# viniciusvidal2/slam-sensor-fusion

Measured on AMD Instinct MI355X. Metric: scans_per_s_200k_scan_vs_10M_map, higher is better.
Workload: dtype f32 points / f64 accumulation

## Files before the change

### include/slamfusion.h

```cpp
#ifndef SLAMFUSION_H
#define SLAMFUSION_H
#include <stdint.h>

#ifdef __cplusplus
extern "C" {
#endif

#define SF_VERSION 210

typedef enum {
    SF_OK = 0,
    SF_ERR_INVALID = -1,
    SF_ERR_HIP = -2,
    SF_ERR_NOMEM = -3,
    SF_ERR_STATE = -4,
    SF_ERR_OVERFLOW = -5,
    SF_ERR_COMM = -6
} sf_status;

typedef struct sf_ctx sf_ctx;
typedef struct sf_cloud sf_cloud;
typedef struct sf_map sf_map;
typedef struct sf_icp sf_icp;

// ... 375 lines not shown
int sf_node_set_coarse_alignment_complete(sf_node *n, int complete);
int sf_node_coarse_alignment_complete(sf_node *n);
sf_icp *sf_node_icp(sf_node *n);
struct sf_bf;
struct sf_bf *sf_node_bf(sf_node *n);

typedef struct sf_ekf sf_ekf;
int sf_ekf_create(sf_ekf **out);
void sf_ekf_destroy(sf_ekf *e);
int sf_ekf_reset(sf_ekf *e, const double T[16], const double v[3] , const double P_diag[9] );
int sf_ekf_set_noise(sf_ekf *e, double gyro_sigma, double accel_sigma, const double gravity[3] );
int sf_ekf_set_bias(sf_ekf *e, const double gyro_bias[3], const double accel_bias[3], const double gyro_bias_var[3], const double accel_bias_var[3]);
int sf_ekf_set_bias_noise(sf_ekf *e, double gyro_bias_walk, double accel_bias_walk);
int sf_ekf_predict_imu(sf_ekf *e, const double *gyro, const double *accel, int64_t n, double dt);
int sf_ekf_predict_odometry(sf_ekf *e, const double odom_T_prev[16], const double odom_T_cur[16], const double cov_pos[3], const double cov_rot[3]);
int sf_ekf_update_position(sf_ekf *e, const double p_map[3], const double cov[9]);
int sf_ekf_update_yaw(sf_ekf *e, double yaw, double var);
int sf_ekf_update_pose(sf_ekf *e, const double T[16], const double cov_pos[3], const double cov_rot[3]);
int sf_ekf_update_pose_cov(sf_ekf *e, const double T[16], const double cov[36]);
int sf_ekf_get(const sf_ekf *e, double T[16], double v[3], double P[81]);
int sf_ekf_get_full(const sf_ekf *e, double gyro_bias[3], double accel_bias[3], double P[225]);

int sf_test_radix_sort(sf_ctx *ctx, int key_bytes , const void *keys, const uint32_t *vals , int64_t n, unsigned end_bit,
                       int lead , int lead_alt , void *keys_out, uint32_t *vals_out , int64_t *guard_damage);
int sf_test_scan_u32(sf_ctx *ctx, int op , const uint32_t *in, int64_t n, uint32_t carry0, int in_place, uint32_t *out,
                     int64_t *guard_damage);

#define SF_TEST_OP_RSQRT 0
#define SF_TEST_OP_SVD3 1
#define SF_TEST_OP_KABSCH 2
#define SF_TEST_OP_LDLT6 3
#define SF_TEST_OP_VEC6 4
#define SF_TEST_OP_JACOBI3 5
#define SF_TEST_OP_JACOBI6 6
#define SF_TEST_OP_ROBUST 7
#define SF_TEST_OP_EIGVEC 8
int sf_test_linalg(sf_ctx *ctx, int op, const double *in, int in_stride, int64_t cases, double *out, int out_stride);
int sf_test_wave_reduce(sf_ctx *ctx, int width , const double *in , double *out );
int sf_test_block_reduce(sf_ctx *ctx, int nrec , const double *in , double *out );
int sf_test_reduce_partials(sf_ctx *ctx, int nrec , int nt , const double *part , int nblocks, double *out );

int sf_test_plane_score(sf_cloud *c, const float *planes, int64_t n_planes, double t, int max_blocks, int64_t *counts);

int sf_test_label_boxes(sf_cloud *c, const int32_t *labels, int64_t n_labels, const sf_box_params *p, int max_blocks,
                        sf_label_box *boxes, sf_box_stats *stats);

#define SF_TEST_SCHEDULE_IN 15
#define SF_TEST_SCHEDULE_OUT 10
int sf_test_launch_schedule(const int32_t *in, int64_t rows, int k, int32_t *out);

int sf_test_compact(sf_cloud *c, const uint8_t *flags);
int sf_test_cloud_minmax(sf_cloud *c, int enqueue_form, float mn[3], float mx[3], int64_t *n_finite);

#ifdef __cplusplus
}
#endif
#endif
```

### slam_sensor_fusion_amd/api.py

```python
import atexit
import ctypes as C
import math
import os
import weakref

import numpy as np

_HERE = os.path.dirname(os.path.abspath(__file__))
LIB_PATH = os.path.join(_HERE, "lib", "libslamfusion.so")

SF_ICP_REF_CPP, SF_ICP_O3D_P2P, SF_ICP_P2PLANE = 0, 1, 2
SF_VOXEL_PCL, SF_VOXEL_O3D, SF_VOXEL_PCL64 = 0, 1, 2
SF_FLAG_VOXEL_OVERFLOW = 1
SF_ICP_FLAG_FEW_CORR, SF_ICP_FLAG_SINGULAR, SF_ICP_FLAG_SHARD_STALE, SF_ICP_FLAG_BARRIER_TIMEOUT = 1, 2, 4, 8
PROF_NN, PROF_REDUCE, PROF_COLLECTIVE, PROF_SOLVE, PROF_SHARD_BUILD = 0, 1, 2, 3, 4
SF_ERR_COMM = -6
MODES = {"ref_cpp": SF_ICP_REF_CPP, "o3d_p2p": SF_ICP_O3D_P2P, "p2plane": SF_ICP_P2PLANE}
ROBUST_KINDS = {"none": 0, "huber": 1, "cauchy": 2, "tukey": 3, "gm": 4}


class SlamFusionError(RuntimeError):
    pass


# ... 130 lines not shown


atexit.register(_close_all)


def load_library():
    global _lib
    if _lib is not None:
        return _lib
    if not os.path.exists(LIB_PATH):
        raise SlamFusionError(
            "libslamfusion.so not found at %s — build it with "
            "`python -c 'import __graft_entry__ as g; g.build()'` (hipcc, gfx950). "
            "There is no CPU fallback." % LIB_PATH)
    try:
        import torch
    except ImportError:
        pass
    lib = C.CDLL(LIB_PATH)
    lib.sf_last_error.restype = C.c_char_p
    lib.sf_ctx_stream.restype = C.c_void_p
    lib.sf_cloud_device_ptr.restype = C.c_void_p
    lib.sf_icp_exchange_ptr.restype = C.c_void_p
    lib.sf_sfilter_create.restype = C.c_void_p
    lib.sf_node_icp.restype = C.c_void_p
    lib.sf_node_bf.restype = C.c_void_p
    lib.sf_fusion_compass_to_yaw.restype = C.c_float
    lib.sf_fusion_closest_altitude.restype = C.c_float
    lib.sf_sfilter_pose_zscore.restype = C.c_float
    lib.sf_icp_set_robust_kernel.argtypes = [C.c_void_p, C.c_int, C.c_double]
    lib.sf_icp_set_covariance.argtypes = [C.c_void_p, C.c_int, C.c_double]
    lib.sf_icp_set_degeneracy_thresholds.argtypes = [C.c_void_p, C.c_double, C.c_double, C.c_double, C.c_double]
    lib.sf_icp_fetch_covariance.argtypes = [C.c_void_p, C.c_void_p]
    lib.sf_icp_fetch_covariance_previous.argtypes = [C.c_void_p, C.c_void_p]
    lib.sf_test_radix_sort.argtypes = [C.c_void_p, C.c_int, C.c_void_p, C.c_void_p, C.c_int64, C.c_uint, C.c_int, C.c_int, C.c_void_p, C.c_void_p, C.c_void_p]
    lib.sf_test_scan_u32.argtypes = [C.c_void_p, C.c_int, C.c_void_p, C.c_int64, C.c_uint32, C.c_int, C.c_void_p, C.c_void_p]
    lib.sf_test_linalg.argtypes = [C.c_void_p, C.c_int, C.c_void_p, C.c_int, C.c_int64, C.c_void_p, C.c_int]
    lib.sf_test_wave_reduce.argtypes = [C.c_void_p, C.c_int, C.c_void_p, C.c_void_p]
    lib.sf_test_block_reduce.argtypes = [C.c_void_p, C.c_int, C.c_void_p, C.c_void_p]
    lib.sf_test_reduce_partials.argtypes = [C.c_void_p, C.c_int, C.c_int, C.c_void_p, C.c_int, C.c_void_p]
    lib.sf_plane_default_params.restype = None
    lib.sf_cloud_plane_hypotheses.argtypes = [C.c_void_p, C.c_void_p, C.c_void_p, C.c_void_p, C.c_void_p]
    lib.sf_cloud_score_planes.argtypes = [C.c_void_p, C.c_void_p, C.c_int64, C.c_double, C.c_void_p]
    lib.sf_cloud_segment_plane.argtypes = [C.c_void_p, C.c_void_p, C.c_void_p, C.c_void_p, C.c_void_p]
    lib.sf_cloud_remove_plane.argtypes = [C.c_void_p, C.c_void_p, C.c_int, C.c_void_p, C.c_void_p]
    lib.sf_test_plane_score.argtypes = [C.c_void_p, C.c_void_p, C.c_int64, C.c_double, C.c_int, C.c_void_p]
    lib.sf_cloud_label_boxes.argtypes = [C.c_void_p, C.c_void_p, C.c_int64, C.c_void_p, C.c_void_p, C.c_void_p]
    lib.sf_test_label_boxes.argtypes = [C.c_void_p, C.c_void_p, C.c_int64, C.c_void_p, C.c_int, C.c_void_p, C.c_void_p]
    lib.sf_cloud_cluster_boxes.argtypes = [C.c_void_p, C.c_double, C.c_int64, C.c_int64, C.c_float, C.c_void_p, C.c_void_p, C.c_int64, C.c_void_p, C.c_void_p]
    lib.sf_cloud_remove_boxes.argtypes = [C.c_void_p, C.c_void_p, C.c_void_p, C.c_void_p, C.c_int64, C.c_double, C.c_int, C.c_void_p]
    lib.sf_test_launch_schedule.argtypes = [C.c_void_p, C.c_int64, C.c_int, C.c_void_p]
    lib.sf_test_compact.argtypes = [C.c_void_p, C.c_void_p]
    lib.sf_test_cloud_minmax.argtypes = [C.c_void_p, C.c_int, C.c_void_p, C.c_void_p, C.c_void_p]
    _lib = lib
    return lib


def voxel_merge_min_points(n=-1):
    return int(load_library().sf_cloud_voxel_merge_min_points(C.c_int64(n)))


def kernel_sources():
    import re
    csrc = os.path.join(_HERE, "csrc")
    found, todo = set(), ["sf_icp.hip"]
    while todo:
        name = todo.pop()
        if name in found or not os.path.isfile(os.path.join(csrc, name)):
            continue
        found.add(name)
        with open(os.path.join(csrc, name), "r", encoding="utf-8", errors="replace") as f:
            todo += re.findall(r'^[ \t]*#[ \t]*include[ \t]*"([^"]+)"', f.read(), re.M)
    return sorted(found)


def kernel_source_hash():
    import hashlib
    h = hashlib.sha256()
    for name in kernel_sources():
        with open(os.path.join(_HERE, "csrc", name), "rb") as f:
            h.update(f.read())
    return h.hexdigest()[:16]


def _check(rc):
    if rc != 0:
        raise SlamFusionError("libslamfusion error %d: %s" % (rc, load_library().sf_last_error().decode()))


def _f32(a):
    return np.ascontiguousarray(a, dtype=np.float32)


def _f64(a):
    return np.ascontiguousarray(a, dtype=np.float64)


def _p(a):
    return a.ctypes.data_as(C.c_void_p)


SCHEDULE_INPUTS = ("mode", "K", "qpl", "sharded", "whole", "reuse", "window", "robust", "wanted", "fz_from", "defer", "table", "nbr_from", "lk_min", "tile_on")
SCHEDULE_OUTPUTS = ("launches", "nn", "one_per_lane", "solve_takes_freeze_state", "ask_freeze", "deferred_rows", "attempt_from", "fz", "lookup_first", "defer_first")
NN_SEARCH, NN_TILE_SEARCH, NN_DEFERRING, NN_FREEZE, NN_FROZEN_FEW = range(5)


# ... 31 lines not shown
def hook_scan_u32(ctx, op, values, carry0=0, in_place=False):
    values = np.ascontiguousarray(values, dtype=np.uint32)
    out = np.empty_like(values)
    damage = C.c_int64(-1)
    _check(ctx.lib.sf_test_scan_u32(ctx.h, int(op), _p(values), len(values), int(carry0), int(bool(in_place)), _p(out), C.addressof(damage)))
    return out, damage.value


LINALG_OPS = {"rsqrt": (0, 1, 2), "svd3": (1, 9, 21), "kabsch": (2, 32, 16), "ldlt6": (3, 42, 7), "vec6": (4, 6, 16),
              "jacobi3": (5, 9, 13), "jacobi6": (6, 36, 43), "robust": (7, 3, 1), "eigvec": (8, 9, 3)}


def hook_linalg(ctx, op, cases):
    code, n_in, n_out = LINALG_OPS[op]
    cases = _f64(cases).reshape(-1, n_in)
    out = np.zeros((len(cases), n_out))
    _check(ctx.lib.sf_test_linalg(ctx.h, code, _p(cases), n_in, len(cases), _p(out), n_out))
    return out


def hook_wave_reduce(ctx, width, values):
    values = _f64(values).reshape(256, int(width))
    out = np.zeros(256)
    _check(ctx.lib.sf_test_wave_reduce(ctx.h, int(width), _p(values), _p(out)))
    return out


def hook_block_reduce(ctx, nrec, values, fill=0.0):
    values = _f64(values).reshape(256, int(nrec))
    out = np.full(32, fill, dtype=np.float64)
    _check(ctx.lib.sf_test_block_reduce(ctx.h, int(nrec), _p(values), _p(out)))
    return out


def hook_reduce_partials(ctx, nrec, nt, part):
    part = _f64(part).reshape(-1, 32)
    out = np.full(32, np.nan)
    _check(ctx.lib.sf_test_reduce_partials(ctx.h, int(nrec), int(nt), _p(part), len(part), _p(out)))
    return out


def hook_compact(cloud, flags):
    flags = np.ascontiguousarray(flags, dtype=np.uint8).reshape(-1)
    if len(flags) != len(cloud):
        raise SlamFusionError("hook_compact: %d flags for %d points" % (len(flags), len(cloud)))
    _check(cloud.lib.sf_test_compact(cloud.h, _p(flags) if len(flags) else None))
    return cloud.download(), cloud.last_indices()


def hook_cloud_minmax(cloud, enqueue=False):
    mn, mx, cnt = np.full(3, np.nan, np.float32), np.full(3, np.nan, np.float32), C.c_int64(-1)
    _check(cloud.lib.sf_test_cloud_minmax(cloud.h, int(bool(enqueue)), _p(mn), _p(mx), C.addressof(cnt)))
    return mn, mx, cnt.value


def _pc2_layout(msg):
    offs, types = {"x": 0, "y": 4, "z": 8}, {"x": 7, "y": 7, "z": 7}
    for f in getattr(msg, "fields", []) or []:
        if f.name in offs:
            offs[f.name] = int(f.offset)
            types[f.name] = int(getattr(f, "datatype", 7))
    if len(set(types.values())) != 1:
        raise SlamFusionError("PointCloud2 x/y/z fields have different datatypes: %r" % (types,))
    buf = np.frombuffer(msg.data, dtype=np.uint8)
    return (buf, int(msg.width), int(msg.height), int(msg.point_step), int(getattr(msg, "row_step", 0) or 0), (offs["x"], offs["y"], offs["z"]), types["x"],
            int(bool(getattr(msg, "is_bigendian", False))))


class Context:

    def __init__(self, device=0, stream=None):
        self.lib = load_library()
        self.h = C.c_void_p()
        _check(self.lib.sf_ctx_create(C.c_int(device), C.c_void_p(stream), C.byref(self.h)))
        _live.add(self)

    def synchronize(self):
        _check(self.lib.sf_ctx_synchronize(self.h))

    @property
    def stream(self):
        return self.lib.sf_ctx_stream(self.h)

    def device_name(self):
        buf = C.create_string_buffer(256)
        _check(self.lib.sf_ctx_device_name(self.h, buf, C.c_int(256)))
        return buf.value.decode()

    def close(self):
        if self.h:
            self.lib.sf_ctx_destroy(self.h)
            self.h = C.c_void_p()

    def __del__(self):
        try:
            self.close()
        except Exception:
            pass


class Cloud:

    def __init__(self, ctx, xyz=None):
        self.ctx, self.lib = ctx, ctx.lib
        self.h = C.c_void_p()
        _check(self.lib.sf_cloud_create(ctx.h, C.byref(self.h)))
# ... 1299 lines not shown
```

### slam_sensor_fusion_amd/csrc/sf_icp.hip

```cpp
#include "sf_common.hpp"
#include "sf_nn.hpp"
#include "sf_tile.hpp"
#include "sf_order.hpp"
#include "sf_p2p.hpp"
#include "sf_schedule.hpp"

#include <cfloat>
#include <cstdlib>
#include <cmath>
#include <vector>
#include <mutex>
#include <string>
#include <type_traits>

namespace {

constexpr int BLK = 256;
constexpr int NREC_P2P = 17;
constexpr int NREC_PLANE = 30;
constexpr int REC_STRIDE = 32;

struct IcpState {
    double T[16];
    double rec[REC_STRIDE];
// ... 736 lines not shown
        const float qx = fmaf(P.T[0], p.x, fmaf(P.T[1], p.y, fmaf(P.T[2], p.z, P.T[3])));
        const float qy = fmaf(P.T[4], p.x, fmaf(P.T[5], p.y, fmaf(P.T[6], p.z, P.T[7])));
        const float qz = fmaf(P.T[8], p.x, fmaf(P.T[9], p.y, fmaf(P.T[10], p.z, P.T[11])));
        if (!(isfinite(qx) && isfinite(qy) && isfinite(qz))) return sf::ORD_KEY_NONE;
        const int cx = sf::grid_cell((qx - g.org[0]) * g.inv_h, g.dim[0]), cy = sf::grid_cell((qy - g.org[1]) * g.inv_h, g.dim[1]),
                  cz = sf::grid_cell((qz - g.org[2]) * g.inv_h, g.dim[2]);
        if (lut) return (uint32_t)lut[order_cell(g, cx, cy, cz) >> lut_shift];
        const uint64_t key = order_cell(g, cx, cy, cz) >> shift;
        return (uint32_t)(key < (uint64_t)(sf::ORD_KEY_NONE - 1u) ? key : (uint64_t)(sf::ORD_KEY_NONE - 1u));
    }
};

__global__ __launch_bounds__(sf::ORD_BLK) void k_order_hist(sf::OrderSrc s, CellKeyFn kf, uint16_t *__restrict__ keys, uint32_t *__restrict__ counts)
{
    sf::order_hist_body(s, kf, keys, counts);
}

constexpr int ORDER_LUT_LOG2 = 16;
__global__ __launch_bounds__(256) void k_order_lut_hist(SfGrid g, int lut_shift, uint32_t *__restrict__ hist)
{
    const int64_t j = (int64_t)blockIdx.x * 256 + threadIdx.x;
    if (j >= g.n) return;
    const float4 p = g.pts[j];
    const int cx = sf::grid_cell((p.x - g.org[0]) * g.inv_h, g.dim[0]), cy = sf::grid_cell((p.y - g.org[1]) * g.inv_h, g.dim[1]),
              cz = sf::grid_cell((p.z - g.org[2]) * g.inv_h, g.dim[2]);
    atomicAdd(&hist[order_cell(g, cx, cy, cz) >> lut_shift], 1u);
}
__global__ __launch_bounds__(1024) void k_order_lut_make(const uint32_t *__restrict__ hist, int nbins, uint32_t n_points, uint16_t *__restrict__ lut)
{
    __shared__ uint32_t part[1024];
    const int per = (nbins + 1023) / 1024, a = (int)threadIdx.x * per, b = min(a + per, nbins);
    uint32_t s = 0;
    for (int k = a; k < b; ++k) s += hist[k];
    part[threadIdx.x] = s;
    __syncthreads();
    for (int o = 1; o < 1024; o <<= 1) {
        const uint32_t v = threadIdx.x >= (unsigned)o ? part[threadIdx.x - o] : 0u;
        __syncthreads();
        part[threadIdx.x] += v;
        __syncthreads();
    }
    uint64_t run = part[threadIdx.x] - s;
    const uint64_t top = (uint64_t)(sf::ORD_KEY_NONE - 1u), n = n_points > 0u ? n_points : 1u;
    for (int k = a; k < b; ++k) {
        const uint64_t key = run * top / n;
        lut[k] = (uint16_t)(key < top ? key : top - 1u);
        run += hist[k];
    }
}

__global__ __launch_bounds__(sf::ORD_BLK) void k_order_scatter(sf::OrderSrc s, const uint16_t *__restrict__ keys, const uint32_t *__restrict__ starts, uint32_t *__restrict__ out)
{
    sf::order_scatter_body(s, keys, starts, out);
}

constexpr int GATHER_PER_LANE = 4;
constexpr int GATHER_TILE = 256 * GATHER_PER_LANE;
__global__ __launch_bounds__(256) void k_order_gather(const float4 *__restrict__ rec, const uint32_t *__restrict__ idx, int64_t total, int seg_n, int seg_tiles, int nseg,
                                                      float *__restrict__ Xx, float *__restrict__ Xy, float *__restrict__ Xz)
{
    int64_t base, end = total;
    if (seg_n > 0) {
        int b, tile;
        if (!sf::order_block(seg_tiles, nseg, &b, &tile)) return;
        base = (int64_t)b * seg_n + (int64_t)tile * GATHER_TILE + threadIdx.x;
        end = (int64_t)(b + 1) * seg_n;
    } else {
        base = (int64_t)blockIdx.x * GATHER_TILE + threadIdx.x;
    }
    uint32_t o[GATHER_PER_LANE];
    float4 v[GATHER_PER_LANE];
#pragma unroll
    for (int k = 0; k < GATHER_PER_LANE; ++k) o[k] = base + 256 * k < end ? idx[base + 256 * k] : 0u;
#pragma unroll
    for (int k = 0; k < GATHER_PER_LANE; ++k) v[k] = rec[o[k]];
#pragma unroll
    for (int k = 0; k < GATHER_PER_LANE; ++k)
        if (base + 256 * k < end) {
            Xx[base + 256 * k] = v[k].x;
            Xy[base + 256 * k] = v[k].y;
            Xz[base + 256 * k] = v[k].z;
        }
}

constexpr uint32_t TILE_KEY_NONE = (1u << 20) - 1u;
struct TileKeyFn {
    SfGrid g;
    sf::SfTiles tl;
    const float *x, *y, *z;
    const IcpState *st;
    int n, digit;
    struct Point { float x, y, z; };
    struct Pose { float T[12]; };
    __device__ __forceinline__ Pose prepare(int b) const
    {
        Pose P;
#pragma unroll
        for (int k = 0; k < 12; ++k) P.T[k] = (float)st[b].T[k];
        return P;
    }
    __device__ __forceinline__ Point load(uint32_t o) const { return Point{x[o], y[o], z[o]}; }
    __device__ __forceinline__ uint32_t full_key(const Pose &P, const Point &p) const
    {
        const float qx = fmaf(P.T[0], p.x, fmaf(P.T[1], p.y, fmaf(P.T[2], p.z, P.T[3])));
        const float qy = fmaf(P.T[4], p.x, fmaf(P.T[5], p.y, fmaf(P.T[6], p.z, P.T[7])));
        const float qz = fmaf(P.T[8], p.x, fmaf(P.T[9], p.y, fmaf(P.T[10], p.z, P.T[11])));
// ... 3421 lines not shown
    prof_collect(icp);
    if (nn_launches) *nn_launches = icp->prof_launches;
    if (nn_ms_total) *nn_ms_total = icp->prof_ms;
    return SF_OK;
}

extern "C" int sf_icp_profile_read_phases(sf_icp *icp, int kind, float *ms, int64_t cap, int64_t *n)
{
    SF_CHECK(icp && kind > 0 && kind < SF_PROF_KINDS, SF_ERR_INVALID, "bad arguments");
    SF_HIP(hipStreamSynchronize(icp->ctx->stream));
    prof_collect(icp);
    const std::vector<float> &v = icp->prof_phase[kind];
    if (n) *n = (int64_t)v.size();
    if (!ms) return SF_OK;
    SF_CHECK(cap >= (int64_t)v.size(), SF_ERR_INVALID, "buffer too small");
    std::memcpy(ms, v.data(), sizeof(float) * v.size());
    return SF_OK;
}

extern "C" int sf_test_linalg(sf_ctx *ctx, int op, const double *in, int in_stride, int64_t cases, double *out, int out_stride)
{
    SF_CHECK(ctx, SF_ERR_INVALID, "sf_test_linalg: ctx is NULL");
    SF_CHECK(op >= 0 && op < TEST_OP_COUNT, SF_ERR_INVALID, "sf_test_linalg: unknown op %d", op);
    SF_CHECK(cases >= 0 && cases <= TEST_MAX_CASES, SF_ERR_INVALID, "sf_test_linalg: cases %lld outside [0, 2^20]", (long long)cases);
    SF_CHECK(in_stride >= TEST_OP_IN[op] && in_stride <= 64 && out_stride >= TEST_OP_OUT[op] && out_stride <= 64, SF_ERR_INVALID,
             "sf_test_linalg: op %d reads %d and writes %d doubles per case (strides %d / %d, at most 64)", op, TEST_OP_IN[op], TEST_OP_OUT[op], in_stride, out_stride);
    SF_CHECK((in && out) || cases == 0, SF_ERR_INVALID, "sf_test_linalg: in or out is NULL");
    if (op == TEST_OP_EIGVEC) return sf::test_map_eigvec(ctx, in, in_stride, cases, out, out_stride);
    return test_linalg_run(ctx, op, in, in_stride, cases, out, out_stride);
}

extern "C" int sf_test_wave_reduce(sf_ctx *ctx, int width, const double *in, double *out)
{
    SF_CHECK(ctx && in && out, SF_ERR_INVALID, "sf_test_wave_reduce: ctx, in or out is NULL");
    SF_CHECK(width == 1 || width == 16 || width == 32, SF_ERR_INVALID, "sf_test_wave_reduce: width %d (1, 16 or 32)", width);
    return test_wave_reduce_run(ctx, width, in, out);
}

extern "C" int sf_test_block_reduce(sf_ctx *ctx, int nrec, const double *in, double *out)
{
    SF_CHECK(ctx && in && out, SF_ERR_INVALID, "sf_test_block_reduce: ctx, in or out is NULL");
    SF_CHECK(nrec == NREC_P2P || nrec == NREC_PLANE, SF_ERR_INVALID, "sf_test_block_reduce: nrec %d (%d or %d)", nrec, NREC_P2P, NREC_PLANE);
    return test_block_reduce_run(ctx, nrec, in, out);
}

extern "C" int sf_test_reduce_partials(sf_ctx *ctx, int nrec, int nt, const double *part, int nblocks, double *out)
{
    SF_CHECK(ctx && out, SF_ERR_INVALID, "sf_test_reduce_partials: ctx or out is NULL");
    SF_CHECK(test_reduce_partials_known(nrec, nt), SF_ERR_INVALID, "sf_test_reduce_partials: <%d, %d> is not an instantiation the library uses (11 | 17 | 24 | 30 by 256, 17 | 30 by 1024)", nrec, nt);
    SF_CHECK(nblocks >= 0 && nblocks <= TEST_MAX_ROWS, SF_ERR_INVALID, "sf_test_reduce_partials: nblocks %d outside [0, 65536]", nblocks);
    SF_CHECK(part || nblocks == 0, SF_ERR_INVALID, "sf_test_reduce_partials: part is NULL");
    return test_reduce_partials_run(ctx, nrec, nt, part, nblocks, out);
}
```

### slam_sensor_fusion_amd/csrc/sf_icp_order_host.hpp

```cpp

namespace {

constexpr int64_t TILE_AUTO_MIN_QUERIES = 2000000;
bool tile_plan(const SfGrid &g, sf::SfTiles *out)
{
    const double ncell = (double)g.dim[0] * (double)g.dim[1] * (double)g.dim[2];
    if (g.n <= 0 || ncell <= 0) return false;
    const double density = (double)g.n / ncell;
    int tc[3] = {8, 8, 4};
    auto region_cells = [&](const int *c) { return (double)(c[0] + 2 * sf::TILE_HALO) * (c[1] + 2 * sf::TILE_HALO) * (c[2] + 2 * sf::TILE_HALO); };
    auto fits_tables = [&](const int *c) { return c[0] + 2 * sf::TILE_HALO <= sf::TILE_RX_MAX && (c[1] + 2 * sf::TILE_HALO) * (c[2] + 2 * sf::TILE_HALO) <= sf::TILE_ROWS_MAX; };
    const double budget = 0.75 * sf::TILE_PCAP;
    while (region_cells(tc) * density > budget) {
        int a = tc[0] >= tc[1] && tc[0] >= tc[2] ? 0 : (tc[1] >= tc[2] ? 1 : 2);
        if (tc[a] <= 2) return false;
        tc[a] /= 2;
    }
    for (;;) {
        int a = tc[2] <= tc[1] && tc[2] <= tc[0] ? 2 : (tc[1] <= tc[0] ? 1 : 0);
        int t2[3] = {tc[0], tc[1], tc[2]};
        t2[a] *= 2;
        if (!fits_tables(t2) || region_cells(t2) * density > budget) break;
        tc[0] = t2[0]; tc[1] = t2[1]; tc[2] = t2[2];
    }
    if (!fits_tables(tc)) return false;
    sf::SfTiles tl;
    int64_t nt = 1;
    for (int a = 0; a < 3; ++a) {
        tl.tc[a] = tc[a];
        tl.nt[a] = (g.dim[a] + tc[a] - 1) / tc[a];
        nt *= tl.nt[a];
    }
    if (nt >= (int64_t)TILE_KEY_NONE) return false;
    tl.ntiles = (int)nt;
    *out = tl;
    return true;
}

bool tile_wanted(const sf_icp *icp, int mode)
{
    const SrcSet &ss = icp->src();
    if (icp->tile_mode == 0 || robust_on(icp, mode) || icp->shard || icp->map->window.kind != 0 || (mode != SF_ICP_P2PLANE && mode != SF_ICP_O3D_P2P)) return false;
    if (ss.qpl == 1) return false;
    return icp->tile_mode == 2 || ss.n * ss.batch >= TILE_AUTO_MIN_QUERIES;
}

constexpr int ORDER_LUT_BINS = (1 << ORDER_LUT_LOG2) + 1;
int order_lut_prepare(sf_icp *icp)
{
    if (!icp->order_lut_on || !icp->map || !icp->map->built) return SF_OK;
    const SfGrid &g = icp->map->grid;
    if (g.n <= 0 || (icp->order_lut.p && icp->order_lut_gen == icp->map->generation)) return SF_OK;
    const OrderSpan sp = order_span(g);
    icp->order_lut_shift = std::max(0, sp.bits - ORDER_LUT_LOG2);
    const int nbins = (int)(sp.cells >> icp->order_lut_shift) + 1;
    SF_TRY(icp->order_lut.reserve(sizeof(uint32_t) * (size_t)ORDER_LUT_BINS + sizeof(uint16_t) * (size_t)ORDER_LUT_BINS));
    uint32_t *hist = icp->order_lut.as<uint32_t>();
    uint16_t *lut = reinterpret_cast<uint16_t *>(hist + ORDER_LUT_BINS);
    hipStream_t st = icp->ctx->stream;
    SF_HIP(hipMemsetAsync(hist, 0, sizeof(uint32_t) * (size_t)ORDER_LUT_BINS, st));
    hipLaunchKernelGGL(k_order_lut_hist, dim3(nblk(g.n)), dim3(256), 0, st, g, icp->order_lut_shift, hist);
    hipLaunchKernelGGL(k_order_lut_make, dim3(1), dim3(1024), 0, st, hist, nbins, (uint32_t)g.n, lut);
    SF_HIP(hipGetLastError());
    icp->order_lut_gen = icp->map->generation;
    return SF_OK;
}

int run_order_sort(sf_icp *icp, int nseg, int64_t longest, int64_t total, const uint32_t *seg_off, const uint32_t *src_idx)
{
    Lane &ln = icp->cur(); SrcSet &ss = icp->src();
    const SfGrid &g = icp->map->grid;
    if (seg_off) icp->tile_on = false;
    sf::OrderSrc src;
    src.src_idx = src_idx;
    src.seg_off = seg_off;
    src.n = (int)ss.n;
    src.tiles = (int)std::max<int64_t>(1, sf::div_up(longest, sf::ORD_TILE));
    CellKeyFn kf;
    kf.g = g;
    kf.x = soa(ss.X0, ss.plane, 0); kf.y = soa(ss.X0, ss.plane, 1); kf.z = soa(ss.X0, ss.plane, 2);
    kf.st = ln.state.as<IcpState>();
    kf.shift = order_key_shift(g);
    kf.lut = nullptr;
    kf.lut_shift = 0;
    if (icp->order_lut_on && icp->order_lut.p && icp->order_lut_gen == icp->map->generation) {
        kf.lut = reinterpret_cast<const uint16_t *>(icp->order_lut.as<uint32_t>() + ORDER_LUT_BINS);
        kf.lut_shift = icp->order_lut_shift;
    }
    const size_t cap = (size_t)std::max<int64_t>(total, 1);
    SF_TRY(ln.Xq.reserve(sizeof(float) * 3 * std::max(cap, (size_t)(seg_off ? 0 : ss.plane))));
    SF_TRY(ln.qkeys.reserve(sizeof(uint16_t) * cap));
    SF_TRY(ln.qkeys2.reserve(sizeof(uint32_t) * (size_t)nseg * (size_t)(src.tiles + 1) * sf::ORD_BINS));
    SF_TRY(ln.qidx.reserve(sizeof(uint32_t) * cap));
    uint16_t *keys = ln.qkeys.as<uint16_t>();
    uint32_t *counts = ln.qkeys2.as<uint32_t>(), *ordered = ln.qidx.as<uint32_t>();
    hipStream_t s = icp->ctx->stream;
    src.nseg = nseg;
    const dim3 grid(sf::order_grid(src.tiles, nseg)), blk(sf::ORD_BLK);
    if (icp->tile_on) {
        TileKeyFn tk;
        tk.g = g; tk.tl = icp->tiles;
        tk.x = kf.x; tk.y = kf.y; tk.z = kf.z;
        tk.st = kf.st; tk.n = (int)ss.n;
        const bool two = icp->tiles.ntiles > sf::ORD_BINS;
        uint32_t *first = ordered;
        if (two) {
            SF_TRY(ln.qidx2.reserve(sizeof(uint32_t) * cap));
            first = ln.qidx2.as<uint32_t>();
        }
        tk.digit = 0;
        hipLaunchKernelGGL(k_order_hist_tile, grid, blk, 0, s, src, tk, keys, counts);
        hipLaunchKernelGGL(sf::k_order_scan, dim3((unsigned)nseg), dim3(sf::ORD_BINS), 0, s, counts, src.tiles);
        hipLaunchKernelGGL(k_order_scatter, grid, blk, 0, s, src, keys, counts, first);
        if (two) {
            sf::OrderSrc src2 = src;
            src2.src_idx = first;
            tk.digit = 1;
            hipLaunchKernelGGL(k_order_hist_tile, grid, blk, 0, s, src2, tk, keys, counts);
            hipLaunchKernelGGL(sf::k_order_scan, dim3((unsigned)nseg), dim3(sf::ORD_BINS), 0, s, counts, src2.tiles);
            hipLaunchKernelGGL(k_order_scatter, grid, blk, 0, s, src2, keys, counts, ordered);
        }
    } else {
        hipLaunchKernelGGL(k_order_hist, grid, blk, 0, s, src, kf, keys, counts);
        hipLaunchKernelGGL(sf::k_order_scan, dim3((unsigned)nseg), dim3(sf::ORD_BINS), 0, s, counts, src.tiles);
        hipLaunchKernelGGL(k_order_scatter, grid, blk, 0, s, src, keys, counts, ordered);
    }
    const int64_t qplane = seg_off ? total : ss.plane;
    if (seg_off) {
        hipLaunchKernelGGL(k_order_gather, dim3(nblk(total, GATHER_TILE)), dim3(256), 0, s, ss.X0r.as<float4>(), ordered, total, 0, 0, 0, soa(ln.Xq, qplane, 0),
                           soa(ln.Xq, qplane, 1), soa(ln.Xq, qplane, 2));
    } else {
        const int gt = (int)std::max<int64_t>(1, sf::div_up(ss.n, GATHER_TILE));
        hipLaunchKernelGGL(k_order_gather, dim3(sf::order_grid(gt, nseg)), dim3(256), 0, s, ss.X0r.as<float4>(), ordered, total, (int)ss.n, gt, nseg,
                           soa(ln.Xq, qplane, 0), soa(ln.Xq, qplane, 1), soa(ln.Xq, qplane, 2));
    }
    if (icp->tile_on) {
        TileKeyFn tk;
        tk.g = g; tk.tl = icp->tiles;
        tk.x = soa(ln.Xq, qplane, 0); tk.y = soa(ln.Xq, qplane, 1); tk.z = soa(ln.Xq, qplane, 2);
        tk.st = kf.st; tk.n = (int)ss.n; tk.digit = 0;
        const int64_t rows = (int64_t)icp->tiles.ntiles + 1;
        SF_TRY(ln.qtkey.reserve(sizeof(uint32_t) * cap));
        SF_TRY(ln.tseg.reserve(sizeof(uint32_t) * (size_t)rows * (size_t)nseg));
        SF_TRY(ln.tile_stats.reserve(sizeof(unsigned long long) * TILE_STATS));
        SF_HIP(hipMemsetAsync(ln.tile_stats.p, 0, sizeof(unsigned long long) * TILE_STATS, s));
        hipLaunchKernelGGL(k_tile_keys, dim3(nblk(total)), dim3(256), 0, s, tk, total, ln.qtkey.as<uint32_t>());
        hipLaunchKernelGGL(k_tile_starts, dim3(nblk(rows * nseg)), dim3(256), 0, s, ln.qtkey.as<uint32_t>(), (int)ss.n, nseg, icp->tiles.ntiles, ln.tseg.as<uint32_t>());
    }
    SF_HIP(hipGetLastError());
    return SF_OK;
// ... 18 lines not shown
```

### slam_sensor_fusion_amd/csrc/sf_order.hpp

```cpp
#pragma once
#include "sf_common.hpp"

namespace sf {

constexpr int ORD_KEY_BITS = 10;
constexpr int ORD_BINS = 1 << ORD_KEY_BITS;
constexpr uint32_t ORD_KEY_NONE = ORD_BINS - 1u;
constexpr int ORD_BLK = 256;
constexpr int ORD_WAVES = ORD_BLK / 64;
constexpr int ORD_PER_LANE = 16;
constexpr int ORD_TILE = ORD_BLK * ORD_PER_LANE;
constexpr int ORD_WAVE_SPAN = 64 * ORD_PER_LANE;

struct OrderSrc {
    const uint32_t *src_idx;
    const uint32_t *seg_off;
    int n;
    int tiles;
    int nseg;
};

__device__ __forceinline__ bool order_block(int tiles, int nseg, int *b, int *tile)
{
    const int lin = blockIdx.x, xcd = lin & 7, k = lin >> 3;
// ... 97 lines not shown
    int b, tile;
    if (!order_block(s.tiles, s.nseg, &b, &tile)) return;
    uint32_t seg_start, seg_len;
    order_segment(s, b, &seg_start, &seg_len);
    if ((uint32_t)tile * ORD_TILE >= seg_len) return;
    const int wv = threadIdx.x >> 6, lane = threadIdx.x & 63;
    for (int d = threadIdx.x; d < ORD_BINS * ORD_WAVES; d += ORD_BLK) (&ctr[0][0])[d] = 0;
    __syncthreads();
    uint32_t key[ORD_PER_LANE];
    bool valid[ORD_PER_LANE];
#pragma unroll
    for (int c = 0; c < ORD_PER_LANE; ++c) {
        const uint32_t e = order_element(tile, c);
        valid[c] = e < seg_len;
        key[c] = valid[c] ? (uint32_t)keys[seg_start + e] : 0u;
    }
#pragma unroll
    for (int c = 0; c < ORD_PER_LANE; ++c)
        if (valid[c]) atomicAdd(&ctr[wv][key[c]], 1u);
    __syncthreads();
    const uint32_t *seg_tab = starts + (size_t)b * (s.tiles + 1) * ORD_BINS;
    for (int d = threadIdx.x; d < ORD_BINS; d += ORD_BLK) {
        uint32_t run = seg_tab[(size_t)tile * ORD_BINS + d] + seg_tab[(size_t)s.tiles * ORD_BINS + d];
#pragma unroll
        for (int w = 0; w < ORD_WAVES; ++w) {
            const uint32_t v = ctr[w][d];
            ctr[w][d] = run;
            run += v;
        }
    }
    __syncthreads();
    const unsigned long long below = (1ull << lane) - 1ull;
    uint32_t rank[ORD_PER_LANE];
#pragma unroll
    for (int c = 0; c < ORD_PER_LANE; ++c) {
        const unsigned long long peers = order_peers(key[c], valid[c]);
        rank[c] = valid[c] ? ctr[wv][key[c]] + (uint32_t)__popcll(peers & below) : 0u;
        __builtin_amdgcn_wave_barrier();
        if (valid[c] && (peers >> lane) <= 1ull) ctr[wv][key[c]] += (uint32_t)__popcll(peers);
        __builtin_amdgcn_fence(__ATOMIC_ACQ_REL, "wavefront");
        __builtin_amdgcn_wave_barrier();
    }
    uint32_t id[ORD_PER_LANE];
#pragma unroll
    for (int c = 0; c < ORD_PER_LANE; ++c) {
        const uint32_t e = order_element(tile, c);
        id[c] = valid[c] ? (s.src_idx ? s.src_idx[seg_start + e] : seg_start + e) : 0u;
    }
#pragma unroll
    for (int c = 0; c < ORD_PER_LANE; ++c)
        if (valid[c]) out[seg_start + rank[c]] = id[c];
}

}
```

Baseline: 22160.

## Fuse order scatter and gather into a single LDS-staged point move kernel

For the plain (untiled, unsegmented) query-ordering path, the ids scatter kernel and the separate gather kernel are replaced by one kernel. It ranks points within the tile, stages each coordinate plane in LDS in sorted order, and writes coalesced runs straight to the ordered point buffers. This drops the intermediate index buffer and the random gather reads. It adds LDS pressure and more barriers per tile, and a test hook compares the new form against the old one.

```diff
diff --git a/include/slamfusion.h b/include/slamfusion.h
--- a/include/slamfusion.h
+++ b/include/slamfusion.h
@@ -451,6 +451,8 @@
 int sf_test_compact(sf_cloud *c, const uint8_t *flags);
 int sf_test_cloud_minmax(sf_cloud *c, int enqueue_form, float mn[3], float mx[3], int64_t *n_finite);
 
+int sf_test_query_order(sf_map *map, const float *points, int batch, int64_t n, const double *poses, int form, int table, uint16_t *keys, float *ordered);
+
 #ifdef __cplusplus
 }
 #endif
diff --git a/slam_sensor_fusion_amd/api.py b/slam_sensor_fusion_amd/api.py
--- a/slam_sensor_fusion_amd/api.py
+++ b/slam_sensor_fusion_amd/api.py
@@ -206,6 +206,7 @@
     lib.sf_test_launch_schedule.argtypes = [C.c_void_p, C.c_int64, C.c_int, C.c_void_p]
     lib.sf_test_compact.argtypes = [C.c_void_p, C.c_void_p]
     lib.sf_test_cloud_minmax.argtypes = [C.c_void_p, C.c_int, C.c_void_p, C.c_void_p, C.c_void_p]
+    lib.sf_test_query_order.argtypes = [C.c_void_p, C.c_void_p, C.c_int, C.c_int64, C.c_void_p, C.c_int, C.c_int, C.c_void_p, C.c_void_p]
     _lib = lib
     return lib
 
@@ -343,6 +344,19 @@
     mn, mx, cnt = np.full(3, np.nan, np.float32), np.full(3, np.nan, np.float32), C.c_int64(-1)
     _check(cloud.lib.sf_test_cloud_minmax(cloud.h, int(bool(enqueue)), _p(mn), _p(mx), C.addressof(cnt)))
     return mn, mx, cnt.value
+
+
+def hook_query_order(map_, points, poses=None, form=1, table=False):
+    points = _f32(points)
+    if points.ndim != 3 or points.shape[2] != 3:
+        raise SlamFusionError("hook_query_order: points must be [B][n][3], not %r" % (points.shape,))
+    batch, n = points.shape[:2]
+    poses = np.tile(np.eye(4), (batch, 1, 1)) if poses is None else _f64(poses).reshape(batch, 4, 4)
+    poses = _f64(poses)
+    keys = np.empty((batch, n), np.uint16)
+    ordered = np.empty((batch, n, 3), np.float32)
+    _check(map_.lib.sf_test_query_order(map_.h, _p(points), batch, n, _p(poses), int(form), int(bool(table)), _p(keys), _p(ordered)))
+    return keys, ordered
 
 
 def _pc2_layout(msg):
diff --git a/slam_sensor_fusion_amd/csrc/sf_icp.hip b/slam_sensor_fusion_amd/csrc/sf_icp.hip
--- a/slam_sensor_fusion_amd/csrc/sf_icp.hip
+++ b/slam_sensor_fusion_amd/csrc/sf_icp.hip
@@ -812,6 +812,13 @@
 __global__ __launch_bounds__(sf::ORD_BLK) void k_order_scatter(sf::OrderSrc s, const uint16_t *__restrict__ keys, const uint32_t *__restrict__ starts, uint32_t *__restrict__ out)
 {
     sf::order_scatter_body(s, keys, starts, out);
+}
+
+__global__ __launch_bounds__(sf::ORD_BLK) void k_order_move(sf::OrderSrc s, const uint16_t *__restrict__ keys, const uint32_t *__restrict__ starts, const float *__restrict__ sx,
+                                                            const float *__restrict__ sy, const float *__restrict__ sz, float *__restrict__ dx, float *__restrict__ dy,
+                                                            float *__restrict__ dz)
+{
+    sf::order_move_body(s, keys, starts, sx, sy, sz, dx, dy, dz);
 }
 
 constexpr int GATHER_PER_LANE = 4;
@@ -4339,3 +4346,64 @@
     SF_CHECK(part || nblocks == 0, SF_ERR_INVALID, "sf_test_reduce_partials: part is NULL");
     return test_reduce_partials_run(ctx, nrec, nt, part, nblocks, out);
 }
+
+extern "C" int sf_test_query_order(sf_map *map, const float *points, int batch, int64_t n, const double *poses, int form, int table, uint16_t *keys, float *ordered)
+{
+    SF_CHECK(map && points && poses && keys && ordered, SF_ERR_INVALID, "sf_test_query_order: a NULL argument");
+    SF_CHECK(map->built && map->grid.n > 0, SF_ERR_INVALID, "sf_test_query_order: the map has no index");
+    SF_CHECK(batch >= 1 && batch <= 64 && n >= 1 && n <= ((int64_t)1 << 20), SF_ERR_INVALID, "sf_test_query_order: batch %d outside [1, 64] or n %lld outside [1, 2^20]", batch,
+             (long long)n);
+    SF_CHECK(form == 0 || form == 1, SF_ERR_INVALID, "sf_test_query_order: form %d (0: ids + gather, 1: the move kernel)", form);
+    sf_ctx *ctx = map->ctx;
+    SF_HIP(hipSetDevice(ctx->device));
+    hipStream_t st = ctx->stream;
+    const size_t total = (size_t)batch * (size_t)n;
+    std::vector<float> h_soa(3 * total);
+    std::vector<float4> h_rec(total);
+    for (size_t i = 0; i < total; ++i) {
+        for (int a = 0; a < 3; ++a) h_soa[(size_t)a * total + i] = points[3 * i + a];
+        h_rec[i] = make_float4(points[3 * i], points[3 * i + 1], points[3 * i + 2], 0.0f);
+    }
+    std::vector<IcpState> h_state((size_t)batch);
+    std::memset(static_cast<void *>(h_state.data()), 0, sizeof(IcpState) * h_state.size());
+    for (int b = 0; b < batch; ++b) std::memcpy(h_state[(size_t)b].T, poses + 16 * (size_t)b, sizeof(double) * 16);
+    sf::OrderSrc src;
+    src.src_idx = nullptr;
+    src.seg_off = nullptr;
+    src.n = (int)n;
+    src.tiles = (int)std::max<int64_t>(1, sf::div_up(n, sf::ORD_TILE));
+    src.nseg = batch;
+    sf::DevBuf x0, rec, state, xq, dkeys, counts, ids, lut;
+    SF_TRY(x0.reserve(sizeof(float) * 3 * total));
+    SF_TRY(rec.reserve(sizeof(float4) * total));
+    SF_TRY(state.reserve(sizeof(IcpState) * (size_t)batch));
+    SF_TRY(xq.reserve(sizeof(float) * 3 * total));
+    SF_TRY(dkeys.reserve(sizeof(uint16_t) * total));
+    SF_TRY(counts.reserve(sizeof(uint32_t) * (size_t)batch * (size_t)(src.tiles + 1) * sf::ORD_BINS));
+    SF_TRY(ids.reserve(sizeof(uint32_t) * total));
+    SF_TRY(sf::upload_staged(ctx, x0.p, h_soa.data(), sizeof(float) * 3 * total));
+    SF_TRY(sf::upload_staged(ctx, rec.p, h_rec.data(), sizeof(float4) * total));
+    SF_TRY(sf::upload_staged(ctx, state.p, h_state.data(), sizeof(IcpState) * (size_t)batch));
+    SF_HIP(hipMemsetAsync(xq.p, 0xff, sizeof(float) * 3 * total, st));
+    CellKeyFn kf;
+    kf.g = map->grid;
+    kf.x = soa(x0, (int64_t)total, 0); kf.y = soa(x0, (int64_t)total, 1); kf.z = soa(x0, (int64_t)total, 2);
+    kf.st = state.as<IcpState>();
+    kf.n = (int)n;
+    kf.shift = order_key_shift(map->grid);
+    kf.lut = nullptr;
+    kf.lut_shift = 0;
+    if (table) {
+        SF_TRY(order_lut_build(st, map->grid, lut, &kf.lut_shift));
+        kf.lut = reinterpret_cast<const uint16_t *>(lut.as<uint32_t>() + ORDER_LUT_BINS);
+    }
+    float *const planes[3] = {soa(xq, (int64_t)total, 0), soa(xq, (int64_t)total, 1), soa(xq, (int64_t)total, 2)};
+    launch_order_plain(st, src, kf, dkeys.as<uint16_t>(), counts.as<uint32_t>(), form, ids.as<uint32_t>(), rec.as<float4>(), planes);
+    SF_HIP(hipGetLastError());
+    SF_HIP(hipMemcpyAsync(keys, dkeys.p, sizeof(uint16_t) * total, hipMemcpyDeviceToHost, st));
+    SF_HIP(hipMemcpyAsync(h_soa.data(), xq.p, sizeof(float) * 3 * total, hipMemcpyDeviceToHost, st));
+    SF_HIP(hipStreamSynchronize(st));
+    for (size_t i = 0; i < total; ++i)
+        for (int a = 0; a < 3; ++a) ordered[3 * i + a] = h_soa[(size_t)a * total + i];
+    return SF_OK;
+}
diff --git a/slam_sensor_fusion_amd/csrc/sf_icp_order_host.hpp b/slam_sensor_fusion_amd/csrc/sf_icp_order_host.hpp
--- a/slam_sensor_fusion_amd/csrc/sf_icp_order_host.hpp
+++ b/slam_sensor_fusion_amd/csrc/sf_icp_order_host.hpp
@@ -46,24 +46,43 @@
 }
 
 constexpr int ORDER_LUT_BINS = (1 << ORDER_LUT_LOG2) + 1;
+int order_lut_build(hipStream_t st, const SfGrid &g, sf::DevBuf &buf, int *shift)
+{
+    const OrderSpan sp = order_span(g);
+    *shift = std::max(0, sp.bits - ORDER_LUT_LOG2);
+    const int nbins = (int)(sp.cells >> *shift) + 1;
+    SF_TRY(buf.reserve(sizeof(uint32_t) * (size_t)ORDER_LUT_BINS + sizeof(uint16_t) * (size_t)ORDER_LUT_BINS));
+    uint32_t *hist = buf.as<uint32_t>();
+    uint16_t *lut = reinterpret_cast<uint16_t *>(hist + ORDER_LUT_BINS);
+    SF_HIP(hipMemsetAsync(hist, 0, sizeof(uint32_t) * (size_t)ORDER_LUT_BINS, st));
+    hipLaunchKernelGGL(k_order_lut_hist, dim3(nblk(g.n)), dim3(256), 0, st, g, *shift, hist);
+    hipLaunchKernelGGL(k_order_lut_make, dim3(1), dim3(1024), 0, st, hist, nbins, (uint32_t)g.n, lut);
+    SF_HIP(hipGetLastError());
+    return SF_OK;
+}
 int order_lut_prepare(sf_icp *icp)
 {
     if (!icp->order_lut_on || !icp->map || !icp->map->built) return SF_OK;
     const SfGrid &g = icp->map->grid;
     if (g.n <= 0 || (icp->order_lut.p && icp->order_lut_gen == icp->map->generation)) return SF_OK;
-    const OrderSpan sp = order_span(g);
-    icp->order_lut_shift = std::max(0, sp.bits - ORDER_LUT_LOG2);
-    const int nbins = (int)(sp.cells >> icp->order_lut_shift) + 1;
-    SF_TRY(icp->order_lut.reserve(sizeof(uint32_t) * (size_t)ORDER_LUT_BINS + sizeof(uint16_t) * (size_t)ORDER_LUT_BINS));
-    uint32_t *hist = icp->order_lut.as<uint32_t>();
-    uint16_t *lut = reinterpret_cast<uint16_t *>(hist + ORDER_LUT_BINS);
-    hipStream_t st = icp->ctx->stream;
-    SF_HIP(hipMemsetAsync(hist, 0, sizeof(uint32_t) * (size_t)ORDER_LUT_BINS, st));
-    hipLaunchKernelGGL(k_order_lut_hist, dim3(nblk(g.n)), dim3(256), 0, st, g, icp->order_lut_shift, hist);
-    hipLaunchKernelGGL(k_order_lut_make, dim3(1), dim3(1024), 0, st, hist, nbins, (uint32_t)g.n, lut);
-    SF_HIP(hipGetLastError());
+    SF_TRY(order_lut_build(icp->ctx->stream, g, icp->order_lut, &icp->order_lut_shift));
     icp->order_lut_gen = icp->map->generation;
     return SF_OK;
+}
+
+void launch_order_plain(hipStream_t s, const sf::OrderSrc &src, const CellKeyFn &kf, uint16_t *keys, uint32_t *counts, int form, uint32_t *ids, const float4 *rec,
+                        float *const xq[3])
+{
+    const dim3 grid(sf::order_grid(src.tiles, src.nseg)), blk(sf::ORD_BLK);
+    hipLaunchKernelGGL(k_order_hist, grid, blk, 0, s, src, kf, keys, counts);
+    hipLaunchKernelGGL(sf::k_order_scan, dim3((unsigned)src.nseg), dim3(sf::ORD_BINS), 0, s, counts, src.tiles);
+    if (form == 1) {
+        hipLaunchKernelGGL(k_order_move, grid, blk, 0, s, src, keys, counts, kf.x, kf.y, kf.z, xq[0], xq[1], xq[2]);
+        return;
+    }
+    hipLaunchKernelGGL(k_order_scatter, grid, blk, 0, s, src, keys, counts, ids);
+    const int gt = (int)std::max<int64_t>(1, sf::div_up(src.n, GATHER_TILE));
+    hipLaunchKernelGGL(k_order_gather, dim3(sf::order_grid(gt, src.nseg)), dim3(256), 0, s, rec, ids, (int64_t)src.n * src.nseg, src.n, gt, src.nseg, xq[0], xq[1], xq[2]);
 }
 
 int run_order_sort(sf_icp *icp, int nseg, int64_t longest, int64_t total, const uint32_t *seg_off, const uint32_t *src_idx)
@@ -91,11 +110,18 @@
     SF_TRY(ln.Xq.reserve(sizeof(float) * 3 * std::max(cap, (size_t)(seg_off ? 0 : ss.plane))));
     SF_TRY(ln.qkeys.reserve(sizeof(uint16_t) * cap));
     SF_TRY(ln.qkeys2.reserve(sizeof(uint32_t) * (size_t)nseg * (size_t)(src.tiles + 1) * sf::ORD_BINS));
-    SF_TRY(ln.qidx.reserve(sizeof(uint32_t) * cap));
     uint16_t *keys = ln.qkeys.as<uint16_t>();
-    uint32_t *counts = ln.qkeys2.as<uint32_t>(), *ordered = ln.qidx.as<uint32_t>();
+    uint32_t *counts = ln.qkeys2.as<uint32_t>();
     hipStream_t s = icp->ctx->stream;
     src.nseg = nseg;
+    if (!icp->tile_on && !seg_off && !src_idx) {
+        float *const xq[3] = {soa(ln.Xq, ss.plane, 0), soa(ln.Xq, ss.plane, 1), soa(ln.Xq, ss.plane, 2)};
+        launch_order_plain(s, src, kf, keys, counts, 1, nullptr, nullptr, xq);
+        SF_HIP(hipGetLastError());
+        return SF_OK;
+    }
+    SF_TRY(ln.qidx.reserve(sizeof(uint32_t) * cap));
+    uint32_t *ordered = ln.qidx.as<uint32_t>();
     const dim3 grid(sf::order_grid(src.tiles, nseg)), blk(sf::ORD_BLK);
     if (icp->tile_on) {
         TileKeyFn tk;
diff --git a/slam_sensor_fusion_amd/csrc/sf_order.hpp b/slam_sensor_fusion_amd/csrc/sf_order.hpp
--- a/slam_sensor_fusion_amd/csrc/sf_order.hpp
+++ b/slam_sensor_fusion_amd/csrc/sf_order.hpp
@@ -173,4 +173,129 @@
         if (valid[c]) out[seg_start + rank[c]] = id[c];
 }
 
-}
+struct OrderMoveLds {
+    union {
+        uint32_t ctr[ORD_WAVES][ORD_BINS];
+        float plane[ORD_TILE];
+    };
+    uint32_t delta[ORD_BINS];
+    uint16_t skey[ORD_TILE];
+    uint32_t wsum[ORD_WAVES];
+};
+static_assert(sizeof(uint32_t) * ORD_WAVES * ORD_BINS == sizeof(float) * ORD_TILE, "the plane takes the counters' place");
+
+__device__ __forceinline__ void order_move_plane(OrderMoveLds &L, const float (&v)[ORD_PER_LANE], const bool (&valid)[ORD_PER_LANE], const uint32_t (&slot)[ORD_PER_LANE],
+                                                 const uint32_t (&pos)[ORD_PER_LANE], uint32_t tile_cnt, float *__restrict__ dst)
+{
+#pragma unroll
+    for (int c = 0; c < ORD_PER_LANE; ++c)
+        if (valid[c]) L.plane[slot[c]] = v[c];
+    __syncthreads();
+    float o[ORD_PER_LANE];
+#pragma unroll
+    for (int j = 0; j < ORD_PER_LANE; ++j) {
+        const uint32_t i = threadIdx.x + (uint32_t)ORD_BLK * j;
+        o[j] = i < tile_cnt ? L.plane[i] : 0.0f;
+    }
+    __syncthreads();
+#pragma unroll
+    for (int j = 0; j < ORD_PER_LANE; ++j)
+        if (threadIdx.x + (uint32_t)ORD_BLK * j < tile_cnt) dst[pos[j]] = o[j];
+}
+
+__device__ __forceinline__ void order_move_body(const OrderSrc &s, const uint16_t *__restrict__ keys, const uint32_t *__restrict__ starts, const float *__restrict__ sx,
+                                                const float *__restrict__ sy, const float *__restrict__ sz, float *__restrict__ dx, float *__restrict__ dy, float *__restrict__ dz)
+{
+    __shared__ OrderMoveLds L;
+    int b, tile;
+    if (!order_block(s.tiles, s.nseg, &b, &tile)) return;
+    const uint32_t seg_len = (uint32_t)s.n, tile_first = (uint32_t)tile * ORD_TILE;
+    if (tile_first >= seg_len) return;
+    const size_t seg_start = (size_t)b * (size_t)s.n;
+    const uint32_t tile_cnt = seg_len - tile_first < (uint32_t)ORD_TILE ? seg_len - tile_first : (uint32_t)ORD_TILE;
+    const int wv = threadIdx.x >> 6, lane = threadIdx.x & 63;
+    for (int d = threadIdx.x; d < ORD_BINS * ORD_WAVES; d += ORD_BLK) (&L.ctr[0][0])[d] = 0;
+    __syncthreads();
+    uint32_t key[ORD_PER_LANE];
+    bool valid[ORD_PER_LANE];
+    float vx[ORD_PER_LANE], vy[ORD_PER_LANE], vz[ORD_PER_LANE];
+#pragma unroll
+    for (int c = 0; c < ORD_PER_LANE; ++c) {
+        const uint32_t e = order_element(tile, c);
+        valid[c] = e < seg_len;
+        key[c] = valid[c] ? (uint32_t)keys[seg_start + e] : 0u;
+    }
+#pragma unroll
+    for (int c = 0; c < ORD_PER_LANE; ++c) vx[c] = valid[c] ? sx[seg_start + order_element(tile, c)] : 0.0f;
+#pragma unroll
+    for (int c = 0; c < ORD_PER_LANE; ++c)
+        if (valid[c]) atomicAdd(&L.ctr[wv][key[c]], 1u);
+    __syncthreads();
+    {
+        static_assert(ORD_BINS == 4 * ORD_BLK, "four buckets per thread");
+        const int d0 = 4 * threadIdx.x;
+        const uint32_t *seg_tab = starts + (size_t)b * (s.tiles + 1) * ORD_BINS;
+        const uint4 tp = *reinterpret_cast<const uint4 *>(seg_tab + (size_t)tile * ORD_BINS + d0);
+        const uint4 bs = *reinterpret_cast<const uint4 *>(seg_tab + (size_t)s.tiles * ORD_BINS + d0);
+        const uint32_t first[4] = {tp.x + bs.x, tp.y + bs.y, tp.z + bs.z, tp.w + bs.w};
+        uint32_t cnt[ORD_WAVES][4], mine = 0;
+#pragma unroll
+        for (int w = 0; w < ORD_WAVES; ++w)
+#pragma unroll
+            for (int j = 0; j < 4; ++j) {
+                cnt[w][j] = L.ctr[w][d0 + j];
+                mine += cnt[w][j];
+            }
+        uint32_t incl = mine;
+#pragma unroll
+        for (int off = 1; off < 64; off <<= 1) {
+            const uint32_t t = __shfl_up(incl, off);
+            if (lane >= off) incl += t;
+        }
+        if (lane == 63) L.wsum[wv] = incl;
+        __syncthreads();
+        uint32_t run = incl - mine;
+#pragma unroll
+        for (int w = 0; w < ORD_WAVES; ++w)
+            if (w < wv) run += L.wsum[w];
+#pragma unroll
+        for (int j = 0; j < 4; ++j) {
+            L.delta[d0 + j] = first[j] - run;
+#pragma unroll
+            for (int w = 0; w < ORD_WAVES; ++w) {
+                L.ctr[w][d0 + j] = run;
+                run += cnt[w][j];
+            }
+        }
+    }
+    __syncthreads();
+    const unsigned long long below = (1ull << lane) - 1ull;
+    uint32_t slot[ORD_PER_LANE];
+#pragma unroll
+    for (int c = 0; c < ORD_PER_LANE; ++c) {
+        const unsigned long long peers = order_peers(key[c], valid[c]);
+        slot[c] = valid[c] ? L.ctr[wv][key[c]] + (uint32_t)__popcll(peers & below) : 0u;
+        __builtin_amdgcn_wave_barrier();
+        if (valid[c] && (peers >> lane) <= 1ull) L.ctr[wv][key[c]] += (uint32_t)__popcll(peers);
+        __builtin_amdgcn_fence(__ATOMIC_ACQ_REL, "wavefront");
+        __builtin_amdgcn_wave_barrier();
+    }
+#pragma unroll
+    for (int c = 0; c < ORD_PER_LANE; ++c) {
+        if (valid[c]) L.skey[slot[c]] = (uint16_t)key[c];
+        vy[c] = valid[c] ? sy[seg_start + order_element(tile, c)] : 0.0f;
+        vz[c] = valid[c] ? sz[seg_start + order_element(tile, c)] : 0.0f;
+    }
+    __syncthreads();
+    uint32_t pos[ORD_PER_LANE];
+#pragma unroll
+    for (int j = 0; j < ORD_PER_LANE; ++j) {
+        const uint32_t i = threadIdx.x + (uint32_t)ORD_BLK * j;
+        pos[j] = i < tile_cnt ? L.delta[L.skey[i]] + i : 0u;
+    }
+    order_move_plane(L, vx, valid, slot, pos, tile_cnt, dx + seg_start);
+    order_move_plane(L, vy, valid, slot, pos, tile_cnt, dy + seg_start);
+    order_move_plane(L, vz, valid, slot, pos, tile_cnt, dz + seg_start);
+}
+
+}
```

Result: faster. 22810 (median of 6 runs) (+2.9%).
